# zhide1983/audio_codec

Measured on AMD Instinct MI355X. Metric: Mframes/s encoded (48kHz/10ms/64kbps), higher is better.
Workload: dtype f32

## Files before the change

### audio_codec_amd/csrc/lc3_enc_rate.inc

```

#ifdef LC3_BIG
#define SHAPE_KERNEL_NAME lc3_enc_shape_kernel_big
#define RATE_KERNEL_NAME  lc3_enc_rate_kernel_big
#define TAILW_KERNEL_NAME lc3_enc_tailw_kernel_big
#define SHAPE_WAVES 3
#ifndef RATE_WAVES_BIG
#define RATE_WAVES_BIG 4
#endif
#define RATE_WAVES RATE_WAVES_BIG
#else
#ifdef LC3_ENC_VBW
#define SHAPE_KERNEL_NAME lc3_enc_shape_kernel_vbw
#else
#define SHAPE_KERNEL_NAME lc3_enc_shape_kernel
#endif
#define RATE_KERNEL_NAME  ERP_FN(lc3_enc_rate_kernel)
#define TAILW_KERNEL_NAME lc3_enc_tailw_kernel
#ifndef SHAPE_WAVES
#define SHAPE_WAVES 4
#endif
#ifndef RATE_WAVES
#define RATE_WAVES 5
#endif
#endif

#ifndef LC3_ENC_RPIPE
struct __attribute__((aligned(16))) ShapeLds {
    static constexpr int MISC = 0;
    static constexpr int XOFF = 0;
    static constexpr int TNS0 = 96, TNS1 = 96 + 184;
    float xbuf[MAXN];
    float A[MAXN];
    float sm[96 + 184 + 80];
    int   pc[LC3D_PLAN_HEAD_WORDS];
    int   cc[14];
    float fsc[12];
    int   isc[56];
#ifdef LC3_STAGE_TIMING
    long long tacc[NSTAGE];
#endif
};

extern "C" __global__ void __launch_bounds__(WAVE) __attribute__((amdgpu_waves_per_eu(SHAPE_WAVES, SHAPE_WAVES)))
SHAPE_KERNEL_NAME(const lc3d_plan* __restrict__ P, const lc3d_chan* __restrict__ chans, int T , int tb, int nt, int fpw, int ncs,
                  float* __restrict__ rows , int srow, float* __restrict__ frec
#ifdef LC3_ENC_VBW
                  , const uint16_t* __restrict__ bwf
#endif
                  )
{
    __shared__ ShapeLds L;
    const int lane = threadIdx.x;
    const int runs = (nt + fpw - 1) / fpw;
    const int cs = blockIdx.x / runs, t0 = tb + (blockIdx.x % runs) * fpw, t1 = imin(tb + nt, t0 + fpw);
    if (cs >= ncs) return;
    if (lane < LC3D_PLAN_HEAD_WORDS) L.pc[lane] = ((const int*)P)[lane];
    if (lane < 14) L.cc[lane] = ((const int*)&chans[cs])[lane];
    if (lane < 56) L.isc[lane] = 0;
    LSYNC();
    const lc3d_chan* __restrict__ C = &chans[cs];
    const int N = PI(N), ylen = PI(ylen);
    constexpr int SPK = (MAXN + WAVE - 1) / WAVE;
    unsigned bob[4] = {0, 0, 0, 0};
#pragma unroll
    for (int k = 0; k < SPK; k++) { const int j = lane + 64 * k; bob[k >> 2] |= (unsigned)(j < N ? P->band_of_bin[j] : 255) << (8 * (k & 3)); }
    float sp[SPK]; float rq = 0; int rb = 0;
#pragma unroll
    for (int k = 0; k < SPK; k++) sp[k] = 0;
#define SHAPE_PREFETCH(t_) do { const float* sr_ = LC3D_ROW_BASE(rows, cs, (t_), T, srow); const float* fr_ = frec + ((size_t)cs * T + (t_)) * FR_WORDS; \
        _Pragma("unroll") for (int k = 0; k < SPK; k++) sp[k] = lane + 64 * k < ylen ? sr_[LC3D_ROW_OFF(lane + 64 * k, T)] : 0.0f; \
        if (lane < 16) rq = fr_[FR_SCFQ + lane]; \
        if (lane == 0) rb = ((const int*)fr_)[FR_BW]; } while (0)
    SHAPE_PREFETCH(t0);
    for (int t = t0; t < t1; t++) {
        float* row = LC3D_ROW_BASE(rows, cs, t, T, srow);
        float* rec = frec + ((size_t)cs * T + t) * FR_WORDS;
#pragma unroll
        for (int k = 0; k < SPK; k++) if (lane + 64 * k < N) XCUR(L)[lane + 64 * k] = sp[k];
        if (lane < 16) L.sm[SM_SCFQ + lane] = rq;
        if (lane == 0) L.isc[I_BW] = rb;
        LSYNC();
        st_sns_apply(P, L, lane, XCUR(L), bob[0], bob[1], bob[2], bob[3]);
#ifdef DUP_SNSAPPLY
        st_sns_apply(P, L, lane, XCUR(L), bob[0], bob[1], bob[2], bob[3]);
#endif
        int bw = uni(L.isc[I_BW]);
#ifdef LC3_ENC_VBW
        const int fbw = bwf[(size_t)(cs / PI(channels)) * T + t];
        if (fbw) {
            const int bin = lc3d_bw_cut_bin(fbw, PI(dms));
            if (ylen > bin) {
                if (lane < 4) { const float sc4[4] = {0.5f, 0.25f, 0.125f, 0.0625f}; L.A[bin - 1 + lane] = L.A[bin - 1 + lane] * sc4[lane]; }
                for (int i = bin + 3 + lane; i < ylen; i += WAVE) L.A[i] = 0;
            }
            bw = imin(bw, lc3d_bw_index(fbw));
        }
#else
        if (CI(bandwidth)) {
            const int bin = CI(bw_cut_bin);
            if (ylen > bin) {
                if (lane < 4) { const float sc4[4] = {0.5f, 0.25f, 0.125f, 0.0625f}; L.A[bin - 1 + lane] = L.A[bin - 1 + lane] * sc4[lane]; }
                for (int i = bin + 3 + lane; i < ylen; i += WAVE) L.A[i] = 0;
            }
            bw = imin(bw, CI(bw_index));
        }
#endif
        const int bw_bin = lc3t_bw_bins[PI(bw_cls) * 6 + bw];
        if (lane < 16) L.isc[I_TNS_IDX0 + lane] = 0;
        if (lane < 2) L.isc[I_TNS_ORD0 + lane] = 0;
        LSYNC();
        st_tns(P, L, lane, bw, bw_bin);
#ifdef DUP_TNS
        st_tns(P, L, lane, bw, bw_bin);
#endif
        st_gain_prep(P, C, L, lane, row, ylen, T, rec);
#ifdef DUP_GAINPREP
        st_gain_prep(P, C, L, lane, row, ylen, T, rec);
#endif
        if (t + 1 < t1) SHAPE_PREFETCH(t + 1);
        for (int i = lane; i < ylen; i += WAVE) row[LC3D_ROW_OFF(i, T)] = L.A[i];
        if (lane < 20) ((int*)rec)[FR_TNS + lane] = L.isc[I_TNS_NF + lane];
        if (lane == 0) ((int*)rec)[FR_BWC] = bw;
        LSYNC();
    }
#undef SHAPE_PREFETCH
}
#endif
#ifndef LC3_ENC_VBW

struct __attribute__((aligned(16))) RateLds {
    uint2    esc[1024];
    uint32_t lut4[1024];
    uint16_t bits[1088];
    int   pc[LC3D_PLAN_HEAD_WORDS];
    int   cc[RATE_WG][14];
};

extern "C" __global__ void __launch_bounds__(RATE_WG * WAVE) __attribute__((amdgpu_waves_per_eu(RATE_WAVES, RATE_WAVES)))
RATE_KERNEL_NAME(const lc3d_plan* __restrict__ P, const lc3d_chan* __restrict__ chans, float* __restrict__ state, int T, int t0, int nt, int ncs,
                 const float* __restrict__ rows , int srow, float* __restrict__ frec ,
                 const float* __restrict__ xnext , int last LC3_ERP_OPT)
{
#ifdef RATE_PRIO
    __builtin_amdgcn_s_setprio(RATE_PRIO);
#endif
    __shared__ RateLds LL;
    const int tid = threadIdx.x, lane = tid & 63, wv = tid >> 6, cs = blockIdx.x * RATE_WG + wv;
    for (int i = tid; i < 1024; i += RATE_WG * WAVE) { LL.esc[i] = ((const uint2*)P->q_esc)[i]; LL.lut4[i] = P->q_lut4[i]; }
    for (int i = tid; i < 1088 / 2; i += RATE_WG * WAVE) ((uint32_t*)LL.bits)[i] = ((const uint32_t*)P->q_bits)[i];
    if (tid < LC3D_PLAN_HEAD_WORDS) LL.pc[tid] = ((const int*)P)[tid];
    if (lane < 14 && cs < ncs) LL.cc[wv][lane] = ((const int*)&chans[cs])[lane];
    LSYNC();
    if (cs >= ncs) return;
#ifdef LC3_ENC_RPIPE
    { const int c = cnt[cs / P->channels]; if (c == 0) return; nt = imax(imin(nt, c - t0), 0); }
#endif
    struct { const int* pc; const int* cc; } L = { LL.pc, LL.cc[wv] };
    float* stp = state + (size_t)cs * LC3D_STATE_WORDS(MEMCAP);
    float tbits_off = unif(stp[LC3D_ST_SCAL(MEMCAP) + F_TBITS_OFF]);
    int mem_target = uni(((const int*)stp)[LC3D_ST_SCAL(MEMCAP) + 16 + I_MEM_TARGET]), mem_spec = uni(((const int*)stp)[LC3D_ST_SCAL(MEMCAP) + 16 + I_MEM_SPEC]);
    const int ylen = PI(ylen), nq = ylen >> 2, half = ylen >> 1, off = CI(gg_off), fs = PI(fs), tb = CI(total_bits);
    const float offs = PI(hrmode) ? 0.5f : 0.375f;
    int rate = 0;
    if ((fs < 48000 && tb > 320 + (fs / 8000 - 2) * 160) || (fs == 48000 && tb > 800)) rate = 512;
    const float thr7 = PF(c_thr7_up), thr50 = PF(c_thr50_dn);
    const float c_lo_f = (float)((2.7) * (28.0 / 20.0));
    const uint32_t* qlut = LL.lut4; const uint2* qesc = LL.esc; const uint16_t* qbits = LL.bits;
    constexpr int NP = (MAXN / 2 + WAVE - 1) / WAVE;
    float2 nx[NP]; float nev[NQL]; int nr = 0; float ng = 0;
#pragma unroll
    for (int k = 0; k < NP; k++) nx[k] = make_float2(0.0f, 0.0f);
#pragma unroll
    for (int h = 0; h < NQL; h++) nev[h] = 0;
#define RATE_PREFETCH(t_) do { const float* sr_ = LC3D_ROW_BASE(rows, cs, (t_), T, srow); const float* fr_ = frec + ((size_t)cs * T + (t_)) * FR_WORDS; \
        _Pragma("unroll") for (int k = 0; k < NP; k++) nx[k] = *(const float2*)&sr_[LC3D_ROW_OFF(2 * imin(lane + 64 * k, half - 1), T)]; \
        _Pragma("unroll") for (int h = 0; h < NQL; h++) nev[h] = sr_[LC3D_ROW_OFF(ylen + imin(lane + 64 * h, nq - 1), T)]; \
        nr = ((const int*)fr_)[lane == 0 ? FR_TNS + 3 : lane == 1 ? FR_LTPF + 3 : FR_XZERO]; \
        ng = fr_[FR_GGMIN]; } while (0)
    if (nt > 0) RATE_PREFETCH(t0);
    for (int t = t0; t < t0 + nt; t++) {
        float2 xv[NP]; float ev[NQL];
#pragma unroll
        for (int k = 0; k < NP; k++) xv[k] = lane + 64 * k < half ? nx[k] : make_float2(0.0f, 0.0f);
#pragma unroll
        for (int h = 0; h < NQL; h++) ev[h] = lane + 64 * h < nq ? nev[h] : 0.0f;
        const int tns_bits = __builtin_amdgcn_readlane(nr, 0), ltpf_bits = __builtin_amdgcn_readlane(nr, 1), xzero = __builtin_amdgcn_readlane(nr, 2);
        const float ind_min = unif(ng);
        const float* en = LC3D_ROW_BASE(rows, cs, t, T, srow);
        float* rec = frec + ((size_t)cs * T + t) * FR_WORDS;
        if (t + 1 < t0 + nt) RATE_PREFETCH(t + 1);
        const int tbq = CI(target_bits_init) - (tns_bits + ltpf_bits);
        if (mem_target < 0) tbits_off = 0;
        else {
            float v = tbits_off + (float)mem_target - (float)mem_spec;
            v = -40 > v ? -40 : v; v = 40 < v ? 40 : v;
            tbits_off = (float)(0.8 * (double)tbits_off + 0.2 * (double)v);
        }
        mem_target = tbq;
        const int nbitsSQ = (int)((double)tbq + round((double)tbits_off));
        float ind = 0;
        if (xzero) mem_target = -1;
        else {
            const float target = (float)((28.0 / 20.0) * (1.4) * (double)nbitsSQ);
            const int offset0 = 255 + off;
            int m = 0;
            for (int i = 0; i < 8; i++) {
                const int fac = 128 >> i, cand = offset0 - m - fac;
                const float fc = (float)cand;
                float tsum = 0; int top = -1;
                bool lo_[NQL]; float tv[NQL];
#pragma unroll
                for (int h = NQL - 1; h >= 0; h--) {
                    const bool valid = lane + 64 * h < nq;
                    const float tt = ev[h] - fc;
                    lo_[h] = !valid || tt < thr7;
                    tv[h] = tt > thr50 ? (tt + tt) - 70.0f : tt;
                    const unsigned long long nz = __ballot(!lo_[h]);
                    if (nz && top < 0) top = 64 * h + 63 - (int)__clzll((long long)nz);
                }
#pragma unroll
                for (int h = 0; h < NQL; h++) tsum += lo_[h] ? (lane + 64 * h < top ? c_lo_f : 0.0f) : tv[h];
                const float S = wave_sum_f_tree(tsum);
                bool addback;
                if (top < 0) addback = false;
                else {
                    const float margin = 4e-5f * S + 1e-4f;
                    if (S - margin > target) addback = true;
                    else if (S + margin < target) addback = false;
                    else addback = gain_probe(thr7, thr50, en, ylen, T, nq, cand, target);
                }
                if (!addback) m += fac;
            }
            const int offset = offset0 - m;
            if ((float)offset < ind_min) mem_target = -1;
            ind = (ind_min > (float)offset ? ind_min : (float)offset) - (float)off;
        }
        const float gain = P->gain_est[uni((int)(ind + (float)off)) + 256];
        const float rgain = 1.0f / gain;
        int q0[NP], q1[NP]; unsigned amb = 0; int lp = 0;
#pragma unroll
        for (int k = 0; k < NP; k++) {
            const float x0 = xv[k].x, x1 = xv[k].y;
            const float v0 = x0 * rgain + copysignf(offs, x0), v1 = x1 * rgain + copysignf(offs, x1);
            q0[k] = (int)v0; q1[k] = (int)v1;
            if (fabsf(v0 - rintf(v0)) <= fabsf(v0) * 5e-7f) amb |= 1u << (2 * k);
            if (fabsf(v1 - rintf(v1)) <= fabsf(v1) * 5e-7f) amb |= 2u << (2 * k);
        }
        if (__ballot(amb != 0)) {
#pragma unroll
            for (int k = 0; k < NP; k++) {
                if ((amb >> (2 * k)) & 1u) { const float x = xv[k].x; q0[k] = (int)truncf(x / gain + copysignf(offs, x)); }
                if ((amb >> (2 * k)) & 2u) { const float x = xv[k].y; q1[k] = (int)truncf(x / gain + copysignf(offs, x)); }
            }
        }
#pragma unroll
        for (int k = 0; k < NP; k++) { const int p = lane + 64 * k; if (p < half && p >= 1 && (q0[k] != 0 || q1[k] != 0)) lp = p; }
        lp = uni(wave_max_i(lp));
        const int lastnz = lp >= 1 ? 2 * lp + 1 : 1;
        const int ntup = (lastnz + 1) >> 1;
        int meta[NP]; unsigned lutw[NP]; uint2 escw[NP]; int ct1 = 0, ct2 = 0;
#pragma unroll
        for (int k = 0; k < NP; k++) {
            meta[k] = 0; lutw[k] = 0; escw[k] = make_uint2(0, 0);
            if (64 * k < ntup) {
                const int p_ = 64 * k + lane; const bool act_ = p_ < ntup;
                const int x0 = act_ ? q0[k] : 0, x1 = act_ ? q1[k] : 0;
                const int a_ = x0 < 0 ? -x0 : x0, b_ = x1 < 0 ? -x1 : x1, mx_ = imax(a_, b_);
                const int nsh = mx_ >= 4 ? ilog2((unsigned)mx_) - 1 : 0;
                const int af_ = a_ >> nsh, bf_ = b_ >> nsh;
                const int lev1 = imin(nsh, 3), s_ = af_ + bf_;
                const int tval_ = lev1 <= 1 ? 1 + (s_ << lev1) : 12 + lev1;
                const int t1_ = dpp_i<DPP_WSHR1>(ct1, tval_), t2_ = dpp_i<DPP_WSHR1>(ct2, t1_);
                ct2 = __builtin_amdgcn_readlane(tval_, 62); ct1 = __builtin_amdgcn_readlane(tval_, 63);
                int tin = 16 * (t2_ & 15) + t1_ + rate; if (2 * p_ > half) tin += 256;
                if (!act_) tin = 0;
                lutw[k] = qlut[tin]; escw[k] = qesc[tin];
                meta[k] = nsh | (lev1 << 5) | ((af_ + 4 * bf_) << 7) | ((imin(a_, 1) + imin(b_, 1)) << 11) | ((act_ ? 1 : 0) << 17);
            }
        }
        int bsum = 0;
#pragma unroll
        for (int k = 0; k < NP; k++) {
            if (64 * k < ntup) {
                const int m_ = meta[k], nsh = m_ & 31, lev1 = (m_ >> 5) & 3, sym = (m_ >> 7) & 15;
                const int pkf = (int)((lutw[k] >> (8 * lev1)) & 255u);
                const int bsym = qbits[pkf * 17 + sym];
                const unsigned w_ = nsh >= 3 ? escw[k].y : escw[k].x;
                const int cv = (int)(nsh == 2 ? w_ >> 16 : w_ & 0xffffu), e3 = (int)(escw[k].y >> 16);
                int bits = nsh == 0 ? 0 : cv + e3 * imax(nsh - 3, 0);
                bits += ((m_ >> 11) & 3) * 2048 + 4096 * nsh + bsym;
                bsum += ((m_ >> 17) & 1) ? bits : 0;
            }
        }
        const int nbits0 = (wave_sum_i(bsum) + 2047) >> 11;
        mem_spec = nbits0;
        if (lane < 4) ((int*)rec)[FR_RATE + lane] = lane == 0 ? (int)ind : lane == 1 ? __float_as_int(gain) : lane == 2 ? nbits0 : lastnz;
    }
#undef RATE_PREFETCH
    if (lane == 0) {
        stp[LC3D_ST_SCAL(MEMCAP) + F_TBITS_OFF] = tbits_off;
        ((int*)stp)[LC3D_ST_SCAL(MEMCAP) + 16 + I_MEM_TARGET] = mem_target; ((int*)stp)[LC3D_ST_SCAL(MEMCAP) + 16 + I_MEM_SPEC] = mem_spec;
    }
    if (last) for (int i = lane; i < MEMCAP; i += WAVE) stp[LC3D_ST_XPREV + i] = xnext[(size_t)cs * MEMCAP + i];
}


#ifndef LC3_ENC_RPIPE
#ifndef TAILW_WAVES
#define TAILW_WAVES 4
#endif
struct __attribute__((aligned(16))) TailwLds {
    static constexpr bool CDW = true;
    static constexpr int MISC = 368;
    static constexpr int XOFF = 0;
    static constexpr int RESO = MAXN / 2, LSTO = MAXN / 2 + 2;
    float xbuf[MAXN];
    float A[MAXN];
    float pad_[2];
    float sm[SMW];
    int   pc[LC3D_PLAN_HEAD_WORDS];
    int   cc[14];
    float fsc[12];
    int   isc[56];
#ifdef LC3_STAGE_TIMING
    long long tacc[NSTAGE];
#endif
};
static_assert(offsetof(TailwLds, A) % 16 == 0 && (offsetof(TailwLds, sm) + (MAXN / 2 + 2) * 4) % 16 == 0, "16-byte aligned LDS rows");

extern "C" __global__ void __launch_bounds__(WAVE) __attribute__((amdgpu_waves_per_eu(TAILW_WAVES, TAILW_WAVES)))
TAILW_KERNEL_NAME(const lc3d_plan* __restrict__ P, const lc3d_chan* __restrict__ chans, int T , int nt, int fpw, int ncs,
                  const float* __restrict__ rows , int srow, const float* __restrict__ frec ,
                  uint8_t* __restrict__ out, int out_stride, uint8_t* __restrict__ status , int min_bytes )
{
    __shared__ TailwLds L;
    const int lane = threadIdx.x;
    const int runs = (nt + fpw - 1) / fpw;
    const int cs = blockIdx.x / runs, t0 = (blockIdx.x % runs) * fpw, t1 = imin(nt, t0 + fpw);
    if (cs >= ncs || chans[cs].nbytes < min_bytes) return;
    if (lane < LC3D_PLAN_HEAD_WORDS) L.pc[lane] = ((const int*)P)[lane];
    if (lane < 14) L.cc[lane] = ((const int*)&chans[cs])[lane];
    if (lane < 56) L.isc[lane] = 0;
    if (lane < 12) L.fsc[lane] = 0;
    LSYNC();
    const lc3d_chan* __restrict__ C = &chans[cs];
    const int ylen = PI(ylen), channels = PI(channels);
    const int strm = cs / channels;
    constexpr int SPK = (MAXN + WAVE - 1) / WAVE;
    float sp[SPK]; int r0 = 0;
#pragma unroll
    for (int k = 0; k < SPK; k++) sp[k] = 0;
#define TAILW_PREFETCH(t_) do { const float* sr_ = LC3D_ROW_BASE(rows, cs, (t_), T, srow); const int* fr_ = (const int*)(frec + ((size_t)cs * T + (t_)) * FR_WORDS); \
        _Pragma("unroll") for (int k = 0; k < SPK; k++) sp[k] = lane + 64 * k < ylen ? sr_[LC3D_ROW_OFF(lane + 64 * k, T)] : 0.0f; \
        r0 = lane < FR_WORDS - FR_IDX ? fr_[FR_IDX + lane] : 0; } while (0)
    TAILW_PREFETCH(t0);
    for (int t = t0; t < t1; t++) {
#pragma unroll
        for (int k = 0; k < SPK; k++) if (lane + 64 * k < MAXN) L.A[lane + 64 * k] = sp[k];
        const int r1 = r0;
        if (lane < 7) L.isc[I_SCF0 + lane] = r1;
        if (lane >= FR_LTPF - FR_IDX && lane < FR_LTPF - FR_IDX + 4) L.isc[I_LTPF0 + lane - (FR_LTPF - FR_IDX)] = r1;
        if (lane >= FR_TNS - FR_IDX && lane < FR_TNS - FR_IDX + 20) L.isc[I_TNS_NF + lane - (FR_TNS - FR_IDX)] = r1;
        if (lane == FR_BWC - FR_IDX) L.isc[I_BW] = r1;
        const int gg0 = __builtin_amdgcn_readlane(r1, FR_RATE - FR_IDX);
        const float gain0 = __int_as_float(__builtin_amdgcn_readlane(r1, FR_RATE - FR_IDX + 1));
        const int gg_min = (int)__int_as_float(__builtin_amdgcn_readlane(r1, FR_GGMIN - FR_IDX));
        if (lane == 0) { L.isc[I_GG] = gg0; L.isc[I_GGMIN] = gg_min; L.fsc[F_GAIN] = gain0; }
        if (t + 1 < t1) TAILW_PREFETCH(t + 1);
        LSYNC();
        const int bw = uni(L.isc[I_BW]);
        const int bw_bin = lc3t_bw_bins[PI(bw_cls) * 6 + bw];
        const int tbq = CI(target_bits_init) - (uni(L.isc[I_TNS_BITS]) + uni(L.isc[I_LTPF_BITS]));
        st_quantize(P, C, L, lane, -1, tbq);
        {
            int gg = gg0, change; float gain = gain0;
            gain_adjust(P, L, gg, gg_min, gain, tbq, uni(L.isc[I_NBITS]), change);
            LSYNC();
            if (lane == 0) { L.isc[I_GG] = gg; L.fsc[F_GAIN] = gain; L.isc[I_CHANGE] = change; }
            LSYNC();
            if (change) st_quantize(P, C, L, lane, 0, tbq);
        }
        st_noise_factor(P, L, lane, bw_bin);
        if (uni(L.isc[I_LSB]) == 0) st_residual(P, L, lane, tbq, uni(L.isc[I_NBITS2]));
        else { for (int i = lane; i < 160; i += WAVE) ((uint32_t*)RESB(L))[i] = 0; if (lane == 0) L.isc[I_NRES] = 0; LSYNC(); }
        if (!PI(hrmode)) {
            const int* xq = XQ(L); const int lastnz = uni(L.isc[I_LASTNZ]);
            bool ovf = false;
            for (int i = lane; i < lastnz; i += WAVE) { const int q = xq[i]; ovf |= q != (int)(int16_t)q; }
            if (status && __ballot(ovf) && lane == 0) status[(size_t)cs * T + t] |= LC3D_ENC_ST_QUANT_RANGE;
        }
        st_bitstream(P, C, L, lane);
        LSYNC();
        if (status && lane == 0 && L.isc[I_BUDGET]) status[(size_t)cs * T + t] |= LC3D_ENC_ST_BIT_BUDGET;
        uint8_t* o = out + ((size_t)strm * T + t) * out_stride + CI(out_off);
        const int nby = CI(nbytes);
        if (((nby | (int)(size_t)o) & 3) == 0) { for (int i = lane; i < (nby >> 2); i += WAVE) ((uint32_t*)o)[i] = ((const uint32_t*)BYTES(L))[i]; }
        else for (int i = lane; i < nby; i += WAVE) o[i] = BYTES(L)[i];
        LSYNC();
    }
#undef TAILW_PREFETCH
}
#endif
#endif
```

Baseline: 113.9.

## Warm-start global gain search from previous frame's offset

Replaces the fixed 8-step bisection of the global gain offset with a hinted search seeded by the previous frame's result. It first probes next to the hint and widens the step exponentially before falling back to bisection. Each probe is a wave reduction and can trigger gain_probe, so fewer probes per frame is meant to cut rate-kernel work. When the hint is poor it can take up to 10 probes, and control flow becomes more data-dependent, which risks divergence and extra overhead.

New measurement: 115.7 (median of 6 runs). 1.5% higher.

```diff
diff --git a/audio_codec_amd/csrc/lc3_enc_rate.inc b/audio_codec_amd/csrc/lc3_enc_rate.inc
--- a/audio_codec_amd/csrc/lc3_enc_rate.inc
+++ b/audio_codec_amd/csrc/lc3_enc_rate.inc
@@ -1,3 +1,8 @@
+
+#ifndef LC3_GS_FN
+#define LC3_GS_FN __device__ __forceinline__
+#endif
+#include "lc3_gain_search.h"
 
 #ifdef LC3_BIG
 #define SHAPE_KERNEL_NAME lc3_enc_shape_kernel_big
@@ -178,6 +183,7 @@
         nr = ((const int*)fr_)[lane == 0 ? FR_TNS + 3 : lane == 1 ? FR_LTPF + 3 : FR_XZERO]; \
         ng = fr_[FR_GGMIN]; } while (0)
     if (nt > 0) RATE_PREFETCH(t0);
+    int hint = LC3_GS_NO_HINT;
     for (int t = t0; t < t0 + nt; t++) {
         float2 xv[NP]; float ev[NQL];
 #pragma unroll
@@ -199,13 +205,11 @@
         mem_target = tbq;
         const int nbitsSQ = (int)((double)tbq + round((double)tbits_off));
         float ind = 0;
-        if (xzero) mem_target = -1;
+        if (xzero) { mem_target = -1; hint = LC3_GS_NO_HINT; }
         else {
             const float target = (float)((28.0 / 20.0) * (1.4) * (double)nbitsSQ);
             const int offset0 = 255 + off;
-            int m = 0;
-            for (int i = 0; i < 8; i++) {
-                const int fac = 128 >> i, cand = offset0 - m - fac;
+            auto probe = [&](int cand) -> int {
                 const float fc = (float)cand;
                 float tsum = 0; int top = -1;
                 bool lo_[NQL]; float tv[NQL];
@@ -221,17 +225,18 @@
 #pragma unroll
                 for (int h = 0; h < NQL; h++) tsum += lo_[h] ? (lane + 64 * h < top ? c_lo_f : 0.0f) : tv[h];
                 const float S = wave_sum_f_tree(tsum);
-                bool addback;
-                if (top < 0) addback = false;
-                else {
-                    const float margin = 4e-5f * S + 1e-4f;
-                    if (S - margin > target) addback = true;
-                    else if (S + margin < target) addback = false;
-                    else addback = gain_probe(thr7, thr50, en, ylen, T, nq, cand, target);
-                }
-                if (!addback) m += fac;
-            }
-            const int offset = offset0 - m;
+                if (top < 0) return 0;
+                const float margin = 4e-5f * S + 1e-4f;
+                if (S - margin > target) return 1;
+                if (S + margin < target) return 0;
+                return uni((int)gain_probe(thr7, thr50, en, ylen, T, nq, cand, target));
+            };
+#ifdef RATE_FULL_BISECT
+            const int offset = lc3_gain_search_bisect(offset0, probe);
+#else
+            const int offset = lc3_gain_search_hinted(offset0, hint, probe);
+            hint = offset;
+#endif
             if ((float)offset < ind_min) mem_target = -1;
             ind = (ind_min > (float)offset ? ind_min : (float)offset) - (float)off;
         }
diff --git a/audio_codec_amd/csrc/lc3_gain_search.h b/audio_codec_amd/csrc/lc3_gain_search.h
--- /dev/null
+++ b/audio_codec_amd/csrc/lc3_gain_search.h
@@ -0,0 +1,49 @@
+#ifndef LC3_GAIN_SEARCH_H
+#define LC3_GAIN_SEARCH_H
+
+#ifndef LC3_GS_FN
+#define LC3_GS_FN inline
+#endif
+
+#define LC3_GS_BISECT_PROBES 8
+#define LC3_GS_MAX_PROBES    10
+#define LC3_GS_NO_HINT       (-0x7fffffff - 1)
+
+template <class Pred> LC3_GS_FN int lc3_gain_search_bisect(int offset0, Pred pred)
+{
+    int m = 0;
+    for (int i = 0; i < LC3_GS_BISECT_PROBES; i++) {
+        const int fac = 128 >> i;
+        if (!pred(offset0 - m - fac)) m += fac;
+    }
+    return offset0 - m;
+}
+
+template <class Pred> LC3_GS_FN int lc3_gain_search_hinted(int offset0, int hint, Pred pred)
+{
+    int a = offset0 - 256, b = offset0;
+    int lim = 1 << (LC3_GS_MAX_PROBES - 1);
+    unsigned steps = 0x84212u;
+    int c = a + 128, last = -1;
+    if (hint == LC3_GS_NO_HINT) steps = 0;
+    else {
+        hint = hint <= a ? a + 1 : hint > b ? b : hint;
+        const int cut = hint - a >= b - hint ? hint - 2 : hint + 1;
+        if (cut > a && cut < b) c = cut; else steps = 0;
+    }
+    for (;;) {
+        const int r = pred(c) ? 1 : 0;
+        a = r ? c : a; b = r ? b : c;
+        const int w = b - a;
+        if (w <= 1) break;
+        if ((last ^ r) == 1) steps = 0;
+        last = r;
+        const int d = (int)(steps & 15u);
+        steps >>= 4; lim >>= 1;
+        c = r ? a + d : b - d;
+        if (d == 0 || (unsigned)(w - d - 1) >= (unsigned)lim) { steps = 0; c = a + (w >> 1); }
+    }
+    return b;
+}
+
+#endif
```
